# bdaiinstitute/vlfm

Hardware: NVIDIA H100
Metric: value-map steps/sec (ITM+cone-fuse) (higher is better)
Workload: dtype f16

## Files before the change

vlfm_b200/csrc/gemm_wgmma.cu:

```cuda
#include <cuda.h>
#include <cuda_fp16.h>
#include <math.h>
#include <stdlib.h>

#include "common.cuh"

namespace vlfm {

constexpr int BM = 128;
constexpr int BK = 64;
constexpr int GEMM_THREADS = 384;
constexpr int GEMM_CONSUMERS = 256;

__device__ __forceinline__ uint32_t smem_u32(const void* p) { return (uint32_t)__cvta_generic_to_shared(p); }

__device__ __forceinline__ void mbar_init(uint32_t bar, uint32_t count) {
  asm volatile("mbarrier.init.shared::cta.b64 [%0], %1;" ::"r"(bar), "r"(count));
}
__device__ __forceinline__ void mbar_expect_tx(uint32_t bar, uint32_t bytes) {
  asm volatile("mbarrier.arrive.expect_tx.shared::cta.b64 _, [%0], %1;" ::"r"(bar), "r"(bytes) : "memory");
}
__device__ __forceinline__ void mbar_arrive(uint32_t bar) {
  asm volatile("mbarrier.arrive.shared::cta.b64 _, [%0];" ::"r"(bar) : "memory");
}
// ... 59 lines not shown
    asm volatile(
        "{\n\t.reg .pred p;\n\tsetp.ne.b32 p, %66, 0;\n\t"
        "wgmma.mma_async.sync.aligned.m64n128k16.f32.f16.f16 "
        "{%0,%1,%2,%3,%4,%5,%6,%7,%8,%9,%10,%11,%12,%13,%14,%15,"
        "%16,%17,%18,%19,%20,%21,%22,%23,%24,%25,%26,%27,%28,%29,%30,%31,"
        "%32,%33,%34,%35,%36,%37,%38,%39,%40,%41,%42,%43,%44,%45,%46,%47,"
        "%48,%49,%50,%51,%52,%53,%54,%55,%56,%57,%58,%59,%60,%61,%62,%63}, %64, %65, p, 1, 1, 0, 0;\n\t}"
        : VLFM_D16(d, 0), VLFM_D16(d, 16), VLFM_D16(d, 32), VLFM_D16(d, 48) : "l"(a), "l"(b), "r"(acc));
  }
};
#undef VLFM_D16
#undef VLFM_D4

struct GemmArgs {
  const float* bias;
  void* out;
  int M, N, K, ldo, epi;
  int kb_per_split;
  long long split_stride;
  const __half* a_tail; int lda, tail_rows, tail_row0;
  void* out_lo;
  int a_box_rows;
  SplitK sk;
};
constexpr int GEMM_TAIL_MAX = 2;
static_assert(SK_SLAB_ROWS == BM + GEMM_TAIL_MAX && SK_TILE == BM, "stream-K slab = one 128 x 128 tile + its tail rows");
constexpr int GEMM_TAIL_KMAX = 6144;

__device__ __forceinline__ float gelu_erf(float x) { return 0.5f * x * (1.f + erff(x * 0.70710678118654752f)); }
__device__ __forceinline__ float silu(float x) { return x / (1.f + expf(-x)); }

__device__ __forceinline__ void epilogue_store2(const GemmArgs& g, int row, int n, float v0, float v1, bool pair, bool split) {
  const size_t idx = (size_t)row * g.ldo + n;
  if (g.epi == VLFM_EPI_BIAS_F16 || g.epi == VLFM_EPI_BIAS_GELU_F16 || g.epi == VLFM_EPI_BIAS_RELU_F16 || g.epi == VLFM_EPI_BIAS_GELU_F16X2) {
    if (g.epi == VLFM_EPI_BIAS_GELU_F16 || g.epi == VLFM_EPI_BIAS_GELU_F16X2) { v0 = gelu_erf(v0); v1 = gelu_erf(v1); }
    else if (g.epi == VLFM_EPI_BIAS_RELU_F16) { v0 = fmaxf(v0, 0.f); v1 = fmaxf(v1, 0.f); }
    __half* o = reinterpret_cast<__half*>(g.out) + idx;
    const __half2 h = __floats2half2_rn(v0, v1);
    if (pair) *reinterpret_cast<__half2*>(o) = h; else o[0] = __low2half(h);
    if (g.epi == VLFM_EPI_BIAS_GELU_F16X2) {
      const float2 f = __half22float2(h);
      const __half2 l = __floats2half2_rn((v0 - f.x) * X2_SCALE, (v1 - f.y) * X2_SCALE);
      __half* ol = reinterpret_cast<__half*>(g.out_lo) + idx;
      if (pair) *reinterpret_cast<__half2*>(ol) = l; else ol[0] = __low2half(l);
    }
  } else {
    const bool partial = (g.epi == VLFM_EPI_PARTIAL_F32);
    float* o = reinterpret_cast<float*>(g.out) + (partial ? (size_t)blockIdx.z * (size_t)g.split_stride : 0) + idx;
    if (split && !partial) {
      atomicAdd(o, v0);
// ... 418 lines not shown
        float2 sum = ld_peer_f2(off, 0);
        for (int p = 1; p < s_cl; ++p) { const float2 v = ld_peer_f2(off, p); sum.x += v.x; sum.y += v.y; }
        epilogue_store2(g, row, n, sum.x + sbias[c], sum.y + sbias[c + 1], n + 1 < g.N, false);
      }
    }
    cluster_sync_all();
  }
}

template <int BN, int STAGES>
__global__ void __launch_bounds__(GEMM_THREADS, 1)
gemm_f16x2_wgmma_kernel(const __grid_constant__ CUtensorMap tmA, const __grid_constant__ CUtensorMap tmAl,
                        const __grid_constant__ CUtensorMap tmB, const __grid_constant__ CUtensorMap tmBl, GemmArgs g) {
  constexpr uint32_t A_BYTES = BM * BK * 2, B_BYTES = BN * BK * 2;

  extern __shared__ uint8_t smem_raw[];
  uint8_t* sA = smem_align_1024(smem_raw);
  uint8_t* sAl = sA + STAGES * A_BYTES;
  uint8_t* sB = sAl + STAGES * A_BYTES;
  uint8_t* sBl = sB + STAGES * B_BYTES;
  uint64_t* bars = reinterpret_cast<uint64_t*>(sBl + STAGES * B_BYTES);
  const uint32_t full0 = smem_u32(bars), empty0 = smem_u32(bars + STAGES);
  float* sbias = reinterpret_cast<float*>(bars + 2 * STAGES);

  pdl_trigger();
  const int warp = threadIdx.x >> 5, lane = threadIdx.x & 31;
  const int n_blk = blockIdx.x, m_blk = blockIdx.y;
  const int kb_begin = blockIdx.z * g.kb_per_split;
  const int num_k = min((g.K + BK - 1) / BK - kb_begin, g.kb_per_split);
  const bool split = gridDim.z > 1;

  if (warp == 0 && lane == 0) {
    asm volatile("prefetch.tensormap [%0];" ::"l"(&tmA) : "memory");
    asm volatile("prefetch.tensormap [%0];" ::"l"(&tmAl) : "memory");
    asm volatile("prefetch.tensormap [%0];" ::"l"(&tmB) : "memory");
    asm volatile("prefetch.tensormap [%0];" ::"l"(&tmBl) : "memory");
    for (int i = 0; i < STAGES; ++i) { mbar_init(full0 + 8 * i, 1); mbar_init(empty0 + 8 * i, GEMM_CONSUMERS / 32); }
    asm volatile("fence.mbarrier_init.release.cluster;" ::: "memory");
    asm volatile("fence.proxy.async.shared::cta;" ::: "memory");
  }
  __syncthreads();

  if (warp == 0) {
    if (lane == 0) {
      const int pre = num_k < STAGES ? num_k : STAGES;
      const uint32_t a_tx = (uint32_t)g.a_box_rows * BK * 2;
      for (int kb = 0; kb < pre; ++kb) {
        mbar_expect_tx(full0 + 8 * kb, 2 * (a_tx + B_BYTES));
        tma_load_2d(smem_u32(sB + kb * B_BYTES), &tmB, (kb_begin + kb) * BK, n_blk * BN, full0 + 8 * kb);
        tma_load_2d(smem_u32(sBl + kb * B_BYTES), &tmBl, (kb_begin + kb) * BK, n_blk * BN, full0 + 8 * kb);
      }
      pdl_wait();
      for (int kb = 0; kb < pre; ++kb) {
        tma_load_2d(smem_u32(sA + kb * A_BYTES), &tmA, (kb_begin + kb) * BK, m_blk * BM, full0 + 8 * kb);
        tma_load_2d(smem_u32(sAl + kb * A_BYTES), &tmAl, (kb_begin + kb) * BK, m_blk * BM, full0 + 8 * kb);
      }
      int s = pre == STAGES ? 0 : pre; uint32_t ph = pre == STAGES ? 1 : 0;
      for (int kb = pre; kb < num_k; ++kb) {
        mbar_wait(empty0 + 8 * s, ph ^ 1);
        mbar_expect_tx(full0 + 8 * s, 2 * (a_tx + B_BYTES));
        tma_load_2d(smem_u32(sA + s * A_BYTES), &tmA, (kb_begin + kb) * BK, m_blk * BM, full0 + 8 * s);
        tma_load_2d(smem_u32(sAl + s * A_BYTES), &tmAl, (kb_begin + kb) * BK, m_blk * BM, full0 + 8 * s);
        tma_load_2d(smem_u32(sB + s * B_BYTES), &tmB, (kb_begin + kb) * BK, n_blk * BN, full0 + 8 * s);
        tma_load_2d(smem_u32(sBl + s * B_BYTES), &tmBl, (kb_begin + kb) * BK, n_blk * BN, full0 + 8 * s);
        if (++s == STAGES) { s = 0; ph ^= 1; }
      }
    }
  } else if (warp >= 4) {
    const int wg = (warp >> 2) - 1, wq = warp & 3;
    const int et = threadIdx.x - (GEMM_THREADS - GEMM_CONSUMERS);
    const int wg_row0 = m_blk * BM + wg * 64;
    const bool active = wg_row0 < g.M;
    if (et < BN) { const int n = n_blk * BN + et; sbias[et] = (g.bias && n < g.N) ? __ldg(g.bias + n) : 0.f; }
    asm volatile("bar.sync 1, 256;" ::: "memory");
    pdl_wait();
    if (!active) {
      int s = 0; uint32_t ph = 0;
      for (int kb = 0; kb < num_k; ++kb) {
        mbar_wait(full0 + 8 * s, ph);
        __syncwarp();
        if (lane == 0) mbar_arrive(empty0 + 8 * s);
        if (++s == STAGES) { s = 0; ph ^= 1; }
      }
      return;
    }
    float acc[BN / 2], corr[BN / 2];
#pragma unroll
    for (int i = 0; i < BN / 2; ++i) { acc[i] = 0.f; corr[i] = 0.f; }
    int s = 0; uint32_t ph = 0;
    for (int kb = 0; kb < num_k; ++kb) {
      mbar_wait(full0 + 8 * s, ph);
// ... 5 lines not shown
      for (int k = 0; k < BK / 16; ++k) {
        const uint64_t da = wgmma_desc_k128(a0 + k * 32), dal = wgmma_desc_k128(al0 + k * 32);
        const uint64_t db = wgmma_desc_k128(b0 + k * 32), dbl = wgmma_desc_k128(bl0 + k * 32);
        const uint32_t first = (kb > 0 || k > 0) ? 1u : 0u;
        Wgmma<BN>::mma(acc, da, db, first);
        Wgmma<BN>::mma(corr, dal, db, first);
        Wgmma<BN>::mma(corr, da, dbl, 1u);
      }
      wg_commit();
      wg_wait<1>();
      if (kb > 0) {
        __syncwarp();
        if (lane == 0) mbar_arrive(empty0 + 8 * (s == 0 ? STAGES - 1 : s - 1));
      }
      if (++s == STAGES) { s = 0; ph ^= 1; }
    }
    wg_wait<0>();
#pragma unroll
    for (int i = 0; i < BN / 2; ++i) acc[i] = fmaf(corr[i], 1.f / X2_SCALE, acc[i]);
    epilogue_frag<BN>(acc, wg_row0 + wq * 16, n_blk, g, split, blockIdx.z == 0, sbias);
  }
}

typedef CUresult (*EncodeTiledFn)(CUtensorMap*, CUtensorMapDataType, cuuint32_t, void*, const cuuint64_t*,
                                  const cuuint64_t*, const cuuint32_t*, const cuuint32_t*, CUtensorMapInterleave,
                                  CUtensorMapSwizzle, CUtensorMapL2promotion, CUtensorMapFloatOOBfill);

static EncodeTiledFn get_encode() {
  static EncodeTiledFn fn = nullptr;
  static bool tried = false;
  if (!tried) {
    tried = true;
    void* p = nullptr;
    cudaDriverEntryPointQueryResult q;
    if (cudaGetDriverEntryPoint("cuTensorMapEncodeTiled", &p, cudaEnableDefault, &q) == cudaSuccess &&
        q == cudaDriverEntryPointSuccess)
      fn = reinterpret_cast<EncodeTiledFn>(p);
  }
  return fn;
}

static int make_map(CUtensorMap* m, const void* base, int rows, int cols, int ld, int boxRows) {
  EncodeTiledFn enc = get_encode();
  if (!enc) { set_error("cuTensorMapEncodeTiled entry point unavailable"); return VLFM_E_DRIVER; }
  cuuint64_t dims[2] = {(cuuint64_t)cols, (cuuint64_t)rows};
  cuuint64_t strides[1] = {(cuuint64_t)ld * 2};
// ... 19 lines not shown
  static_assert(smem <= 227 * 1024, "GEMM stage ring exceeds the 227 KB a block may use");
  static bool configured = false;
  if (!configured) {
    rc = check_cuda(cudaFuncSetAttribute(gemm_f16_wgmma_kernel<BN, STAGES, SILU>, cudaFuncAttributeMaxDynamicSharedMemorySize, (int)smem), "cudaFuncSetAttribute(gemm)");
    if (rc) return rc;
    configured = true;
  }
  const int num_k = (g.K + BK - 1) / BK;
  dim3 grid((g.N + BN - 1) / BN, g.tail_rows > 0 ? g.M / BM : (g.M + BM - 1) / BM, (num_k + g.kb_per_split - 1) / g.kb_per_split);
  if (g.sk.ctas > 0) grid = dim3(g.sk.ctas);
  rc = check_cuda(launch_pdl(gemm_f16_wgmma_kernel<BN, STAGES, SILU>, grid, dim3(GEMM_THREADS), smem, st, ta, tb, g), "gemm_f16_wgmma_kernel");
  if (rc) return rc;
  count_launch();
  return VLFM_OK;
}


template <int BN, int STAGES>
static int launch_gemm_x2(const CUtensorMap& ta, const CUtensorMap& tal, const void* W, const void* Wl, int ldw, const GemmArgs& g, cudaStream_t st) {
  CUtensorMap tb, tbl;
  int rc = make_map(&tb, W, g.N, g.K, ldw, BN);
  if (!rc) rc = make_map(&tbl, Wl, g.N, g.K, ldw, BN);
  if (rc) return rc;
  constexpr size_t smem = (size_t)STAGES * 2 * (BM * BK * 2 + BN * BK * 2) + 2 * STAGES * 8 + 1024 + BN * 4;
  static_assert(smem <= 227 * 1024, "x2 GEMM stage ring exceeds the 227 KB a block may use");
  static bool configured = false;
  if (!configured) {
    rc = check_cuda(cudaFuncSetAttribute(gemm_f16x2_wgmma_kernel<BN, STAGES>, cudaFuncAttributeMaxDynamicSharedMemorySize, (int)smem), "cudaFuncSetAttribute(gemm x2)");
    if (rc) return rc;
    configured = true;
  }
  const int num_k = (g.K + BK - 1) / BK;
  dim3 grid((g.N + BN - 1) / BN, (g.M + BM - 1) / BM, (num_k + g.kb_per_split - 1) / g.kb_per_split);
  rc = check_cuda(launch_pdl(gemm_f16x2_wgmma_kernel<BN, STAGES>, grid, dim3(GEMM_THREADS), smem, st, ta, tal, tb, tbl, g), "gemm_f16x2_wgmma_kernel");
  if (rc) return rc;
  count_launch();
  return VLFM_OK;
}

template <int BN, int STAGES>
struct Csplit {
  static constexpr size_t smem = (size_t)STAGES * (CS_BM * BK * 2 + BN * BK * 2) + 2 * STAGES * 8 + 1024 + BN * 4 +
                                 (size_t)GEMM_TAIL_MAX * GEMM_TAIL_KMAX * 2;
  static_assert(smem <= 227 * 1024, "cluster-split GEMM stage ring exceeds the 227 KB a block may use");
  static int configure() {
    static int rc = -1;
    if (rc < 0) rc = check_cuda(cudaFuncSetAttribute(gemm_f16_csplit_wgmma_kernel<BN, STAGES>, cudaFuncAttributeMaxDynamicSharedMemorySize, (int)smem),
                                "cudaFuncSetAttribute(gemm csplit)");
    return rc;
  }
  static int max_clusters(int s) {
    static int fit[9] = {-1, -1, -1, -1, -1, -1, -1, -1, -1};
    if (fit[s] < 0) {
      fit[s] = 0;
      if (configure()) return 0;
      cudaLaunchConfig_t cfg{};
      cfg.gridDim = dim3(s); cfg.blockDim = dim3(CS_THREADS); cfg.dynamicSmemBytes = smem;
      cudaLaunchAttribute attr[1];
      attr[0].id = cudaLaunchAttributeClusterDimension;
      attr[0].val.clusterDim.x = s; attr[0].val.clusterDim.y = 1; attr[0].val.clusterDim.z = 1;
      cfg.attrs = attr; cfg.numAttrs = 1;
      int n = 0;
      if (cudaOccupancyMaxActiveClusters(&n, gemm_f16_csplit_wgmma_kernel<BN, STAGES>, &cfg) == cudaSuccess) fit[s] = n;
      else cudaGetLastError();
    }
    return fit[s];
  }
  static int launch(const CUtensorMap& ta, const void* W, int ldw, const GemmArgs& g, int s, cudaStream_t st) {
    CUtensorMap tb;
    int rc = make_map(&tb, W, g.N, g.K, ldw, BN);
    if (!rc) rc = configure();
    if (rc) return rc;
    cudaLaunchConfig_t cfg{};
    cfg.gridDim = dim3(((g.N + BN - 1) / BN) * s); cfg.blockDim = dim3(CS_THREADS); cfg.dynamicSmemBytes = smem; cfg.stream = st;
    cudaLaunchAttribute attr[2];
    attr[0].id = cudaLaunchAttributeClusterDimension;
    attr[0].val.clusterDim.x = s; attr[0].val.clusterDim.y = 1; attr[0].val.clusterDim.z = 1;
    attr[1].id = cudaLaunchAttributeProgrammaticStreamSerialization;
    attr[1].val.programmaticStreamSerializationAllowed = 1;
    cfg.attrs = attr; cfg.numAttrs = pdl_enabled() ? 2 : 1;
    rc = check_cuda(cudaLaunchKernelEx(&cfg, gemm_f16_csplit_wgmma_kernel<BN, STAGES>, ta, tb, g), "gemm_f16_csplit_wgmma_kernel");
    if (rc) return rc;
    count_launch();
    return VLFM_OK;
  }
};

}

using namespace vlfm;

static int gemm_dispatch(const void* d_A, const void* d_W, int M, int N, int K, int lda, int ldw, GemmArgs g, void* stream, float* d_partials,
                         size_t partial_bytes, SplitK* layout, bool csplit);

static int sm_count() {
  static int sms = 0;
  if (!sms) { int dev = 0; cudaGetDevice(&dev); if (cudaDeviceGetAttribute(&sms, cudaDevAttrMultiProcessorCount, dev) != cudaSuccess || sms < 1) sms = 132; }
  return sms;
}

extern "C" int vlfm_gemm_f16(const void* d_A, const void* d_W, const float* d_bias, void* d_out, int M, int N,
                             int K, int lda, int ldw, int ldo, int epilogue, void* stream) {
  if (!d_A || !d_W || !d_out || M < 1 || N < 1 || K < 1) { set_error("vlfm_gemm_f16: bad argument"); return VLFM_E_INVALID; }
  if ((K & 7) || (lda & 7) || (ldw & 7) || (ldo & 7) || ((uintptr_t)d_A & 15) || ((uintptr_t)d_W & 15) || ((uintptr_t)d_out & 15)) {
    set_error("vlfm_gemm_f16: K, lda, ldw, ldo must be multiples of 8 and pointers 16-byte aligned"); return VLFM_E_INVALID; }
  const bool csplit = (epilogue & VLFM_EPI_CLUSTER_SPLIT) != 0 && (epilogue & ~VLFM_EPI_CLUSTER_SPLIT) != VLFM_EPI_BIAS_SILU_F16;
  epilogue &= ~VLFM_EPI_CLUSTER_SPLIT;
// ... 154 lines not shown
                   int rows, int D, int ldx, int ldo16, int ldo32, float eps, void* stream);
namespace vlfm {
int layernorm_reduce_impl(float* d_x, const float* d_partials, const SplitK& sk, const float* d_gamma, const float* d_beta, void* d_out16,
                          void* d_out16_lo, float* d_out32, int rows, int D, int ldx, int ldo16, int ldo32, float eps, void* stream);
}

extern "C" int vlfm_gemm_f16_resid_ln(const void* d_A, const void* d_W, const float* d_bias, float* d_x, int M, int N, int K,
                                      int lda, int ldw, int ldx, const float* d_gamma, const float* d_beta, void* d_out16,
                                      int ld16, float* d_out32, int ld32, float eps, float* d_partials, size_t partial_bytes, void* stream) {
  if (!d_A || !d_W || !d_x || !d_gamma || !d_beta || (!d_out16 && !d_out32) || M < 1 || N < 1 || K < 1) {
    set_error("vlfm_gemm_f16_resid_ln: bad argument"); return VLFM_E_INVALID; }
  if ((K & 7) || (lda & 7) || (ldw & 7) || (ldx & 7) || (N & 3) || (ld16 & 3) || (ld32 & 3) || ((uintptr_t)d_A & 15) || ((uintptr_t)d_W & 15) ||
      ((uintptr_t)d_x & 15) || ((uintptr_t)d_partials & 15)) { set_error("vlfm_gemm_f16_resid_ln: alignment (K, strides %% 8; N %% 4; 16-byte pointers)"); return VLFM_E_INVALID; }
  int rc = layernorm_check("vlfm_gemm_f16_resid_ln", d_x, d_gamma, d_beta, d_out16, nullptr, d_out32, N, ldx, ld16, ld32);
  if (rc) return rc;
  GemmArgs g{d_bias, d_x, M, N, K, ldx, VLFM_EPI_BIAS_RESID_F32, (K + BK - 1) / BK, 0, nullptr, 0, 0, 0, nullptr, BM};
  SplitK layout;
  rc = gemm_dispatch(d_A, d_W, M, N, K, lda, ldw, g, stream, d_partials, partial_bytes, &layout, d_partials != nullptr);
  if (rc) return rc;
  if (layout.splits != 1) return layernorm_reduce_impl(d_x, d_partials, layout, d_gamma, d_beta, d_out16, nullptr, d_out32, M, N, ldx, ld16, ld32, eps, stream);
  return vlfm_layernorm(d_x, d_gamma, d_beta, d_out16, d_out32, M, N, ldx, ld16, ld32, eps, stream);
}

static int gemm_x2_dispatch(const void* d_A_hi, const void* d_A_lo, const void* d_W_hi, const void* d_W_lo, int M, int N, int K, int lda, int ldw,
                            GemmArgs g, void* stream, float* d_partials, size_t partial_bytes, int* splits_out) {
  if (splits_out) *splits_out = 1;
  const int rem = M % BM;
  if (M > BM && rem >= 1 && rem <= 32 && (g.epi == VLFM_EPI_BIAS_F32 || g.epi == VLFM_EPI_BIAS_GELU_F16X2)) {
    const int m0 = M - rem;
    GemmArgs g0 = g; g0.M = m0;
    int rc0 = gemm_x2_dispatch(d_A_hi, d_A_lo, d_W_hi, d_W_lo, m0, N, K, lda, ldw, g0, stream, nullptr, 0, nullptr);
    if (rc0) return rc0;
    GemmArgs g1 = g; g1.M = rem;
    const size_t esz = g.epi == VLFM_EPI_BIAS_F32 ? 4 : 2;
    g1.out = (uint8_t*)g.out + (size_t)m0 * g.ldo * esz;
    if (g.out_lo) g1.out_lo = (uint8_t*)g.out_lo + (size_t)m0 * g.ldo * 2;
    return gemm_x2_dispatch((const __half*)d_A_hi + (size_t)m0 * lda, (const __half*)d_A_lo + (size_t)m0 * lda, d_W_hi, d_W_lo, rem, N, K, lda, ldw, g1,
                            stream, nullptr, 0, nullptr);
  }
  CUtensorMap ta, tal;
  g.a_box_rows = M <= 32 ? 32 : (M <= 64 ? 64 : BM);
  int rc = make_map(&ta, d_A_hi, M, K, lda, g.a_box_rows);
  if (!rc) rc = make_map(&tal, d_A_lo, M, K, lda, g.a_box_rows);
  if (rc) return rc;
  const int mt = (M + BM - 1) / BM, num_k = (K + BK - 1) / BK;
  int bn = 32;
  if (mt >= 2 && N >= 4096) bn = 128;
  else if ((long)mt * ((N + 63) / 64) >= 96) bn = 64;
  const int tiles = mt * ((N + bn - 1) / bn);
  int sp = 1;
  if (g.epi == VLFM_EPI_BIAS_RESID_F32 && d_partials) {
    sp = sm_count() / tiles; if (sp > num_k / 3) sp = num_k / 3; if (sp > 8) sp = 8; if (sp < 1) sp = 1;
  }
  g.kb_per_split = (num_k + sp - 1) / sp;
  const int launched = (num_k + g.kb_per_split - 1) / g.kb_per_split;
  if (launched > 1) {
    if ((size_t)launched * (size_t)M * (size_t)N * 4 > partial_bytes) { g.kb_per_split = num_k; }
    else { g.epi = VLFM_EPI_PARTIAL_F32; g.out = d_partials; g.ldo = N; g.split_stride = (long long)M * N; if (splits_out) *splits_out = launched; }
  }
  cudaStream_t st = (cudaStream_t)stream;
  if (bn == 128) return launch_gemm_x2<128, 3>(ta, tal, d_W_hi, d_W_lo, ldw, g, st);
  if (bn == 64) return launch_gemm_x2<64, 4>(ta, tal, d_W_hi, d_W_lo, ldw, g, st);
  return launch_gemm_x2<32, 5>(ta, tal, d_W_hi, d_W_lo, ldw, g, st);
}

static int x2_args_ok(const char* who, const void* a, const void* al, const void* w, const void* wl, const void* out, int M, int N, int K, int lda, int ldw, int ldo) {
  if (!a || !al || !w || !wl || !out || M < 1 || N < 1 || K < 1) { set_error("%s: bad argument", who); return VLFM_E_INVALID; }
  if ((K & 7) || (lda & 7) || (ldw & 7) || (ldo & 7) || ((uintptr_t)a & 15) || ((uintptr_t)al & 15) || ((uintptr_t)w & 15) || ((uintptr_t)wl & 15) || ((uintptr_t)out & 15)) {
// ... 39 lines not shown
```

vlfm_b200/csrc/vit_ops.cu:

```cuda
#include <cuda_fp16.h>
#include <math.h>

#include "common.cuh"

namespace vlfm {

__device__ __forceinline__ uint8_t clip8(int v) {
  v >>= 22;
  return (uint8_t)(v < 0 ? 0 : (v > 255 ? 255 : v));
}

__global__ void resize_h_kernel(const uint8_t* __restrict__ in, uint8_t* __restrict__ mid, int H, int W, int OW,
                                const int* __restrict__ bounds, const int* __restrict__ kk, int ksize) {
  const int b = blockIdx.z, y = blockIdx.y;
  const int i = blockIdx.x * blockDim.x + threadIdx.x;
  if (i >= OW * 3) return;
  const int xo = i / 3, c = i - 3 * xo;
  const int x0 = bounds[2 * xo], n = bounds[2 * xo + 1];
  const uint8_t* row = in + ((size_t)b * H + y) * W * 3;
  int ss = 1 << 21;
  for (int t = 0; t < n; ++t) ss += (int)row[(x0 + t) * 3 + c] * kk[xo * ksize + t];
  mid[(((size_t)b * H + y) * OW + xo) * 3 + c] = clip8(ss);
}

// ... 433 lines not shown
    const float4 v = reinterpret_cast<const float4*>(src)[i];
    __half h[4], l[4];
    split_x2(v.x, h[0], l[0]); split_x2(v.y, h[1], l[1]); split_x2(v.z, h[2], l[2]); split_x2(v.w, h[3], l[3]);
    if (hi) reinterpret_cast<uint2*>(hi)[i] = *reinterpret_cast<uint2*>(h);
    reinterpret_cast<uint2*>(lo)[i] = *reinterpret_cast<uint2*>(l);
  }
}

constexpr int ATT32_NKMAX = 272;
constexpr int ATT32_KT = (ATT32_NKMAX + 31) / 32;
template <int HD>
__global__ void __launch_bounds__(256)
attention_f32_kernel(const float* __restrict__ q, const float* __restrict__ k, const float* __restrict__ v, __half* __restrict__ o_hi,
                     __half* __restrict__ o_lo, int ldq, int ldk, int ldv, int ldo, int Nq, int Nk, float scale) {
  extern __shared__ float sm32[];
  pdl_trigger();
  const int h = blockIdx.x, b = blockIdx.y, warp = threadIdx.x >> 5, lane = threadIdx.x & 31;
  constexpr int KP = HD + 1, HD4 = HD / 4, NC = HD / 32;
  float* sK = sm32;
  float* sV = sK + (((size_t)Nk * KP + 3) & ~(size_t)3);
  float* sQ = sV + (size_t)Nk * HD;
  float* sP = sQ + 8 * HD;
  pdl_wait();
  const int total = Nk * HD4;
#pragma unroll 4
  for (int i = threadIdx.x; i < total; i += 256) {
    const int j = i / HD4, c = (i - j * HD4) << 2;
    const float4 kv = __ldg(reinterpret_cast<const float4*>(k + (size_t)(b * Nk + j) * ldk + h * HD + c));
    const float4 vv = __ldg(reinterpret_cast<const float4*>(v + (size_t)(b * Nk + j) * ldv + h * HD + c));
    float* kd = sK + (size_t)j * KP + c;
    kd[0] = kv.x; kd[1] = kv.y; kd[2] = kv.z; kd[3] = kv.w;
    *reinterpret_cast<float4*>(sV + (size_t)j * HD + c) = vv;
  }
  __syncthreads();
  float* myq = sQ + warp * HD;
  float* myp = sP + (size_t)warp * Nk;
  const int kt = (Nk + 31) >> 5;
  for (int r = blockIdx.z * 8 + warp; r < Nq; r += gridDim.z * 8) {
    const float* qr = q + (size_t)(b * Nq + r) * ldq + h * HD;
#pragma unroll
    for (int c = 0; c < NC; ++c) myq[lane + 32 * c] = qr[lane + 32 * c];
    __syncwarp();
    float sc[ATT32_KT];
    const float* kr[ATT32_KT];
#pragma unroll
    for (int t = 0; t < ATT32_KT; ++t) { sc[t] = 0.f; kr[t] = sK + (size_t)min(lane + 32 * t, Nk - 1) * KP; }
#pragma unroll 4
    for (int d = 0; d < HD; ++d) {
      const float qd = myq[d];
#pragma unroll
      for (int t = 0; t < ATT32_KT; ++t) if (t < kt) sc[t] = fmaf(qd, kr[t][d], sc[t]);
    }
    float mx = -INFINITY;
#pragma unroll
    for (int t = 0; t < ATT32_KT; ++t) {
      sc[t] = (lane + 32 * t < Nk) ? sc[t] * scale : -INFINITY;
      mx = fmaxf(mx, sc[t]);
    }
#pragma unroll
    for (int o = 16; o; o >>= 1) mx = fmaxf(mx, __shfl_xor_sync(0xffffffffu, mx, o));
    float sum = 0.f;
#pragma unroll
    for (int t = 0; t < ATT32_KT; ++t) {
      const float e = (lane + 32 * t < Nk) ? expf(sc[t] - mx) : 0.f;
// ... 237 lines not shown
```

vlfm_b200/vlm/blip2_engine.py:

```python
from __future__ import annotations

import ctypes
import math
import os
from typing import Dict, List, Sequence, Tuple

import numpy as np
import torch

from .. import _lib
from . import dense
from .blip2_config import Blip2Dims
from .preprocess import CLIP_MEAN, CLIP_STD, bicubic_tables

F16, F32 = torch.float16, torch.float32


def partials_floats(dims: Blip2Dims, max_batch: int) -> int:
    rows = max_batch * dims.tokens
    return max(8 * min(rows, 1024), 3 * rows) * max(dims.v_hidden, dims.q_hidden)


class Blip2ITCEngine:
    def __init__(self, dims: Blip2Dims, state_dict: Dict[str, torch.Tensor], device="cuda", max_batch: int = 1,
# ... 158 lines not shown
        hb, hk, hks, vb, vk, vks = self._resize_tables(Hh, Ww)
        rc = self.lib.vlfm_preprocess_im2col(img.data_ptr(), mid.data_ptr(), self.b_col.data_ptr(), B, Hh, Ww, d.image, d.image,
                                             d.patch, d.patch_k_padded, hb.data_ptr(), hk.data_ptr(), hks, vb.data_ptr(),
                                             vk.data_ptr(), vks, self._mean, self._std, _lib.stream_ptr())
        _lib.check(rc, "vlfm_preprocess_im2col")
        self._gemm(self.b_col[: B * (T - 1)], self.patch_w, self.patch_b, _lib.EPI_BIAS_F32, self.b_patch[: B * (T - 1)])
        rc = self.lib.vlfm_assemble_tokens(self.b_patch.data_ptr(), self.cls.data_ptr(), self.pos.data_ptr(), self.b_x.data_ptr(),
                                           B, T, D, _lib.stream_ptr())
        _lib.check(rc, "vlfm_assemble_tokens")
        x, xn, qkv, ao, hb_ = self.b_x[:n], self.b_xn[:n], self.b_qkv[:n], self.b_ao[:n], self.b_h[:n]
        hd = D // d.v_heads
        img16, img32 = self.b_img[:n], self.b_img32[:n]
        dense.layernorm(x, self.vit[0]["ln1_w"], self.vit[0]["ln1_b"], d.v_eps, xn)
        for i, L in enumerate(self.vit):
            self._gemm(xn, L["qkv_w"], L["qkv_b"], _lib.EPI_BIAS_F16, qkv)
            dense.attention_f16(qkv[:, 0:D], qkv[:, D : 2 * D], qkv[:, 2 * D : 3 * D], B, d.v_heads, T, T, hd, hd**-0.5, ao)
            self._gemm_resid_ln(ao, L["proj_w"], L["proj_b"], x, L["ln2_w"], L["ln2_b"], xn, None, d.v_eps)
            self._gemm(xn, L["fc1_w"], L["fc1_b"], _lib.EPI_BIAS_GELU_F16, hb_)
            if i + 1 < len(self.vit):
                nx = self.vit[i + 1]
                self._gemm_resid_ln(hb_, L["fc2_w"], L["fc2_b"], x, nx["ln1_w"], nx["ln1_b"], xn, None, d.v_eps)
            else:
                self._gemm_resid_ln(hb_, L["fc2_w"], L["fc2_b"], x, self.post_w, self.post_b, img16, img32, d.v_eps)
        img_lo = self.b_img_lo[:n]
        dense.split_x2(img32, img_lo)
        kv = self.b_kv32[:n]
        self._gemm_x2(img16, img_lo, self.kv_w, self.kv_wl, self.kv_b, _lib.EPI_BIAS_F32, kv)
        h32, hhi, hlo = self.q_h32[:nq], self.q_h16[:nq], self.q_h_lo[:nq]
        h32.copy_(self.f0_32x[:nq])
        self._qformer_layers(h32, hhi, hlo, B, Q, kv, T, text=False)
        self._gemm_x2(hhi, hlo, self.vp_w, self.vp_wl, self.vp_b, _lib.EPI_BIAS_F32, self.q_proj[:nq])
        rc = self.lib.vlfm_itc_head(self.q_proj.data_ptr(), self.text_feat.data_ptr(), self.out.data_ptr(), B, Q, d.proj,
                                    _lib.stream_ptr())
        _lib.check(rc, "vlfm_itc_head")

    def _fold_layer0(self) -> None:
        d = self.d
        Q, H = d.queries, d.q_hidden
        hd = H // d.q_heads
        L = self.qf[0]
        with torch.cuda.device(self.dev):
            h32 = torch.empty(Q, H, dtype=F32, device=self.dev)
            hhi, hlo = torch.empty(Q, H, dtype=F16, device=self.dev), torch.empty(Q, H, dtype=F16, device=self.dev)
            dense.layernorm_x2(self.query_tokens, self.q_ln_w, self.q_ln_b, d.q_eps, hhi, hlo, h32)
            qkv, ahi, alo = self.q_qkv32[:Q], self.q_ao[:Q], self.q_ao_lo[:Q]
            self._gemm_x2(hhi, hlo, L["qkv_w"], L["qkv_wl"], L["qkv_b"], _lib.EPI_BIAS_F32, qkv)
# ... 99 lines not shown
```

Baseline: 227.6.

## Add cluster-split x2 GEMM for small M and fuse tail rows into x2 kernel

Adds a cluster-split K-parallel two-term fp16 (x2) GEMM kernel for M ≤ 64, which reduces partial sums across the cluster through distributed shared memory. It also lets idle producer-group warps in the main x2 kernel compute 1–2 leftover tail rows with CUDA-core FMAs, replacing a separate launch for the remainder rows. The attention kernel now loads the first query row before the K/V staging loop so that load overlaps the staging. The cost is more shared memory per block and extra mbarrier arrivals on the tail CTAs.

```diff
diff --git a/vlfm_b200/csrc/gemm_wgmma.cu b/vlfm_b200/csrc/gemm_wgmma.cu
--- a/vlfm_b200/csrc/gemm_wgmma.cu
+++ b/vlfm_b200/csrc/gemm_wgmma.cu
@@ -105,10 +105,12 @@
   void* out_lo;
   int a_box_rows;
   SplitK sk;
+  const __half* a_tail_lo;
 };
 constexpr int GEMM_TAIL_MAX = 2;
 static_assert(SK_SLAB_ROWS == BM + GEMM_TAIL_MAX && SK_TILE == BM, "stream-K slab = one 128 x 128 tile + its tail rows");
 constexpr int GEMM_TAIL_KMAX = 6144;
+constexpr int X2_TAIL_KMAX = 1536;
 
 __device__ __forceinline__ float gelu_erf(float x) { return 0.5f * x * (1.f + erff(x * 0.70710678118654752f)); }
 __device__ __forceinline__ float silu(float x) { return x / (1.f + expf(-x)); }
@@ -573,6 +575,7 @@
   uint64_t* bars = reinterpret_cast<uint64_t*>(sBl + STAGES * B_BYTES);
   const uint32_t full0 = smem_u32(bars), empty0 = smem_u32(bars + STAGES);
   float* sbias = reinterpret_cast<float*>(bars + 2 * STAGES);
+  __half* sx = reinterpret_cast<__half*>(sbias + BN);
 
   pdl_trigger();
   const int warp = threadIdx.x >> 5, lane = threadIdx.x & 31;
@@ -580,13 +583,14 @@
   const int kb_begin = blockIdx.z * g.kb_per_split;
   const int num_k = min((g.K + BK - 1) / BK - kb_begin, g.kb_per_split);
   const bool split = gridDim.z > 1;
+  const bool tail_cta = g.tail_rows > 0 && m_blk == (int)gridDim.y - 1;
 
   if (warp == 0 && lane == 0) {
     asm volatile("prefetch.tensormap [%0];" ::"l"(&tmA) : "memory");
     asm volatile("prefetch.tensormap [%0];" ::"l"(&tmAl) : "memory");
     asm volatile("prefetch.tensormap [%0];" ::"l"(&tmB) : "memory");
     asm volatile("prefetch.tensormap [%0];" ::"l"(&tmBl) : "memory");
-    for (int i = 0; i < STAGES; ++i) { mbar_init(full0 + 8 * i, 1); mbar_init(empty0 + 8 * i, GEMM_CONSUMERS / 32); }
+    for (int i = 0; i < STAGES; ++i) { mbar_init(full0 + 8 * i, 1); mbar_init(empty0 + 8 * i, GEMM_CONSUMERS / 32 + (tail_cta ? 3 : 0)); }
     asm volatile("fence.mbarrier_init.release.cluster;" ::: "memory");
     asm volatile("fence.proxy.async.shared::cta;" ::: "memory");
   }
@@ -617,7 +621,70 @@
         if (++s == STAGES) { s = 0; ph ^= 1; }
       }
     }
-  } else if (warp >= 4) {
+  } else if (warp < 4) {
+    if (!tail_cta) return;
+    const int t = threadIdx.x - 32, kpad = num_k * BK;
+    pdl_wait();
+    for (int i = t; i < g.tail_rows * 2 * (kpad >> 3); i += 96) {
+      const int rr = i / (kpad >> 3), c8 = (i - rr * (kpad >> 3)) << 3;
+      uint4 xv = make_uint4(0u, 0u, 0u, 0u);
+      if (c8 < g.K) xv = __ldg(reinterpret_cast<const uint4*>(((rr & 1) ? g.a_tail_lo : g.a_tail) + (size_t)(rr >> 1) * g.lda + c8));
+      *reinterpret_cast<uint4*>(sx + (size_t)rr * kpad + c8) = xv;
+    }
+    asm volatile("bar.sync 2, 96;" ::: "memory");
+    float tm[2][GEMM_TAIL_MAX], tc[2][GEMM_TAIL_MAX];
+#pragma unroll
+    for (int j = 0; j < 2; ++j)
+#pragma unroll
+      for (int r = 0; r < GEMM_TAIL_MAX; ++r) { tm[j][r] = 0.f; tc[j][r] = 0.f; }
+    int s = 0; uint32_t ph = 0;
+    for (int kb = 0; kb < num_k; ++kb) {
+      mbar_wait(full0 + 8 * s, ph);
+#pragma unroll
+      for (int j = 0; j < 2; ++j) {
+        const int f = t + 96 * j;
+        if (f >= BN) continue;
+        const uint8_t* wh_row = sB + (size_t)s * B_BYTES + (size_t)f * 128;
+        const uint8_t* wl_row = sBl + (size_t)s * B_BYTES + (size_t)f * 128;
+#pragma unroll 2
+        for (int c = 0; c < 8; ++c) {
+          const uint4 wh = *reinterpret_cast<const uint4*>(wh_row + ((c ^ (f & 7)) << 4));
+          const uint4 wl = *reinterpret_cast<const uint4*>(wl_row + ((c ^ (f & 7)) << 4));
+          const __half2* whh = reinterpret_cast<const __half2*>(&wh);
+          const __half2* wlh = reinterpret_cast<const __half2*>(&wl);
+#pragma unroll
+          for (int r = 0; r < GEMM_TAIL_MAX; ++r) {
+            if (r < g.tail_rows) {
+              const uint4 xh = *reinterpret_cast<const uint4*>(sx + (size_t)(2 * r) * kpad + kb * BK + c * 8);
+              const uint4 xl = *reinterpret_cast<const uint4*>(sx + (size_t)(2 * r + 1) * kpad + kb * BK + c * 8);
+              const __half2* xhh = reinterpret_cast<const __half2*>(&xh);
+              const __half2* xlh = reinterpret_cast<const __half2*>(&xl);
+#pragma unroll
+              for (int e = 0; e < 4; ++e) {
+                const float2 ah = __half22float2(xhh[e]), al = __half22float2(xlh[e]);
+                const float2 bh = __half22float2(whh[e]), bl = __half22float2(wlh[e]);
+                tm[j][r] = fmaf(ah.x, bh.x, tm[j][r]); tm[j][r] = fmaf(ah.y, bh.y, tm[j][r]);
+                tc[j][r] = fmaf(al.x, bh.x, tc[j][r]); tc[j][r] = fmaf(ah.x, bl.x, tc[j][r]);
+                tc[j][r] = fmaf(al.y, bh.y, tc[j][r]); tc[j][r] = fmaf(ah.y, bl.y, tc[j][r]);
+              }
+            }
+          }
+        }
+      }
+      __syncwarp();
+      if (lane == 0) mbar_arrive(empty0 + 8 * s);
+      if (++s == STAGES) { s = 0; ph ^= 1; }
+    }
+#pragma unroll
+    for (int j = 0; j < 2; ++j) {
+      const int f = t + 96 * j, n = n_blk * BN + f;
+      if (f >= BN || n >= g.N) continue;
+      const float b = g.bias ? __ldg(g.bias + n) : 0.f;
+#pragma unroll
+      for (int r = 0; r < GEMM_TAIL_MAX; ++r)
+        if (r < g.tail_rows) epilogue_store2(g, g.tail_row0 + r, n, fmaf(tc[j][r], 1.f / X2_SCALE, tm[j][r]) + b, 0.f, false, false);
+    }
+  } else {
     const int wg = (warp >> 2) - 1, wq = warp & 3;
     const int et = threadIdx.x - (GEMM_THREADS - GEMM_CONSUMERS);
     const int wg_row0 = m_blk * BM + wg * 64;
@@ -669,6 +736,136 @@
   }
 }
 
+constexpr int CX_THREADS = 256;
+constexpr int CX_ROWS = 64;
+
+template <int BN, int STAGES>
+__global__ void __launch_bounds__(CX_THREADS, 1)
+gemm_f16x2_csplit_wgmma_kernel(const __grid_constant__ CUtensorMap tmA, const __grid_constant__ CUtensorMap tmAl,
+                         const __grid_constant__ CUtensorMap tmB, const __grid_constant__ CUtensorMap tmBl, GemmArgs g) {
+  constexpr uint32_t A_BYTES = CX_ROWS * BK * 2, B_BYTES = BN * BK * 2;
+  constexpr int LDP = BN + 8;
+  static_assert((size_t)CX_ROWS * LDP * 4 <= (size_t)STAGES * 2 * (A_BYTES + B_BYTES), "partial tile must fit the ring");
+
+  extern __shared__ uint8_t smem_raw[];
+  uint8_t* sA = smem_align_1024(smem_raw);
+  uint8_t* sAl = sA + STAGES * A_BYTES;
+  uint8_t* sB = sAl + STAGES * A_BYTES;
+  uint8_t* sBl = sB + STAGES * B_BYTES;
+  uint64_t* bars = reinterpret_cast<uint64_t*>(sBl + STAGES * B_BYTES);
+  const uint32_t full0 = smem_u32(bars), empty0 = smem_u32(bars + STAGES);
+  float* sbias = reinterpret_cast<float*>(bars + 2 * STAGES);
+  float* part = reinterpret_cast<float*>(sA);
+
+  pdl_trigger();
+  const int warp = threadIdx.x >> 5, lane = threadIdx.x & 31;
+  const int nk = (g.K + BK - 1) / BK;
+  const int s_cl = (int)cluster_nctarank(), rank = (int)cluster_ctarank();
+  const int n_blk = blockIdx.x / s_cl;
+  const int kb_lo = rank * nk / s_cl, kb_hi = (rank + 1) * nk / s_cl;
+
+  if (warp == 0 && lane == 0) {
+    asm volatile("prefetch.tensormap [%0];" ::"l"(&tmA) : "memory");
+    asm volatile("prefetch.tensormap [%0];" ::"l"(&tmAl) : "memory");
+    asm volatile("prefetch.tensormap [%0];" ::"l"(&tmB) : "memory");
+    asm volatile("prefetch.tensormap [%0];" ::"l"(&tmBl) : "memory");
+    for (int i = 0; i < STAGES; ++i) { mbar_init(full0 + 8 * i, 1); mbar_init(empty0 + 8 * i, 4); }
+    asm volatile("fence.mbarrier_init.release.cluster;" ::: "memory");
+    asm volatile("fence.proxy.async.shared::cta;" ::: "memory");
+  }
+  __syncthreads();
+
+  if (warp < 4) {
+    if (warp == 0 && lane == 0) {
+      const int pre = min(kb_hi - kb_lo, STAGES);
+      const uint32_t tx = 2 * ((uint32_t)g.a_box_rows * BK * 2 + B_BYTES);
+      for (int i = 0; i < pre; ++i) {
+        mbar_expect_tx(full0 + 8 * i, tx);
+        tma_load_2d(smem_u32(sB + i * B_BYTES), &tmB, (kb_lo + i) * BK, n_blk * BN, full0 + 8 * i);
+        tma_load_2d(smem_u32(sBl + i * B_BYTES), &tmBl, (kb_lo + i) * BK, n_blk * BN, full0 + 8 * i);
+      }
+      pdl_wait();
+      for (int i = 0; i < pre; ++i) {
+        tma_load_2d(smem_u32(sA + i * A_BYTES), &tmA, (kb_lo + i) * BK, 0, full0 + 8 * i);
+        tma_load_2d(smem_u32(sAl + i * A_BYTES), &tmAl, (kb_lo + i) * BK, 0, full0 + 8 * i);
+      }
+      int s = pre == STAGES ? 0 : pre; uint32_t ph = pre == STAGES ? 1 : 0;
+      for (int kb = kb_lo + pre; kb < kb_hi; ++kb) {
+        mbar_wait(empty0 + 8 * s, ph ^ 1);
+        mbar_expect_tx(full0 + 8 * s, tx);
+        tma_load_2d(smem_u32(sA + s * A_BYTES), &tmA, kb * BK, 0, full0 + 8 * s);
+        tma_load_2d(smem_u32(sAl + s * A_BYTES), &tmAl, kb * BK, 0, full0 + 8 * s);
+        tma_load_2d(smem_u32(sB + s * B_BYTES), &tmB, kb * BK, n_blk * BN, full0 + 8 * s);
+        tma_load_2d(smem_u32(sBl + s * B_BYTES), &tmBl, kb * BK, n_blk * BN, full0 + 8 * s);
+        if (++s == STAGES) { s = 0; ph ^= 1; }
+      }
+    }
+    __syncwarp();
+  } else {
+    const int wq = warp & 3, et = threadIdx.x - 128;
+    if (et < BN) { const int n = n_blk * BN + et; sbias[et] = (g.bias && n < g.N) ? __ldg(g.bias + n) : 0.f; }
+    asm volatile("bar.sync 1, 128;" ::: "memory");
+    pdl_wait();
+    float acc[BN / 2], corr[BN / 2];
+#pragma unroll
+    for (int i = 0; i < BN / 2; ++i) { acc[i] = 0.f; corr[i] = 0.f; }
+    int s = 0; uint32_t ph = 0;
+    for (int kb = kb_lo; kb < kb_hi; ++kb) {
+      mbar_wait(full0 + 8 * s, ph);
+      const uint32_t a0 = smem_u32(sA + s * A_BYTES), al0 = smem_u32(sAl + s * A_BYTES);
+      const uint32_t b0 = smem_u32(sB + s * B_BYTES), bl0 = smem_u32(sBl + s * B_BYTES);
+      wg_fence();
+#pragma unroll
+      for (int k = 0; k < BK / 16; ++k) {
+        const uint64_t da = wgmma_desc_k128(a0 + k * 32), dal = wgmma_desc_k128(al0 + k * 32);
+        const uint64_t db = wgmma_desc_k128(b0 + k * 32), dbl = wgmma_desc_k128(bl0 + k * 32);
+        const uint32_t first = (kb > kb_lo || k > 0) ? 1u : 0u;
+        Wgmma<BN>::mma(acc, da, db, first);
+        Wgmma<BN>::mma(corr, dal, db, first);
+        Wgmma<BN>::mma(corr, da, dbl, 1u);
+      }
+      wg_commit();
+      wg_wait<1>();
+      if (kb > kb_lo) {
+        __syncwarp();
+        if (lane == 0) mbar_arrive(empty0 + 8 * (s == 0 ? STAGES - 1 : s - 1));
+      }
+      if (++s == STAGES) { s = 0; ph ^= 1; }
+    }
+    wg_wait<0>();
+#pragma unroll
+    for (int i = 0; i < BN / 2; ++i) acc[i] = fmaf(corr[i], 1.f / X2_SCALE, acc[i]);
+    if (s_cl == 1) {
+      epilogue_frag<BN>(acc, wq * 16, n_blk, g, false, true, sbias);
+    } else {
+      asm volatile("bar.sync 1, 128;" ::: "memory");
+      const int r_up = wq * 16 + (lane >> 2), cq = (lane & 3) * 2;
+#pragma unroll
+      for (int j = 0; j < BN / 8; ++j) {
+        *reinterpret_cast<float2*>(part + r_up * LDP + j * 8 + cq) = make_float2(acc[4 * j], acc[4 * j + 1]);
+        *reinterpret_cast<float2*>(part + (r_up + 8) * LDP + j * 8 + cq) = make_float2(acc[4 * j + 2], acc[4 * j + 3]);
+      }
+    }
+  }
+  if (s_cl > 1) {
+    cluster_sync_all();
+    if (warp >= 4) {
+      const int et = threadIdx.x - 128;
+      const int r0 = rank * g.M / s_cl, r1 = (rank + 1) * g.M / s_cl;
+      const uint32_t base = smem_u32(part);
+      for (int i = et; i < (r1 - r0) * (BN / 2); i += 128) {
+        const int row = r0 + i / (BN / 2), c = (i % (BN / 2)) * 2, n = n_blk * BN + c;
+        if (n >= g.N) continue;
+        const uint32_t off = base + (uint32_t)(row * LDP + c) * 4;
+        float2 sum = ld_peer_f2(off, 0);
+        for (int p = 1; p < s_cl; ++p) { const float2 v = ld_peer_f2(off, p); sum.x += v.x; sum.y += v.y; }
+        epilogue_store2(g, row, n, sum.x + sbias[c], sum.y + sbias[c + 1], n + 1 < g.N, false);
+      }
+    }
+    cluster_sync_all();
+  }
+}
+
 typedef CUresult (*EncodeTiledFn)(CUtensorMap*, CUtensorMapDataType, cuuint32_t, void*, const cuuint64_t*,
                                   const cuuint64_t*, const cuuint32_t*, const cuuint32_t*, CUtensorMapInterleave,
                                   CUtensorMapSwizzle, CUtensorMapL2promotion, CUtensorMapFloatOOBfill);
@@ -734,7 +931,8 @@
   int rc = make_map(&tb, W, g.N, g.K, ldw, BN);
   if (!rc) rc = make_map(&tbl, Wl, g.N, g.K, ldw, BN);
   if (rc) return rc;
-  constexpr size_t smem = (size_t)STAGES * 2 * (BM * BK * 2 + BN * BK * 2) + 2 * STAGES * 8 + 1024 + BN * 4;
+  constexpr size_t smem = (size_t)STAGES * 2 * (BM * BK * 2 + BN * BK * 2) + 2 * STAGES * 8 + 1024 + BN * 4 +
+                          (size_t)2 * GEMM_TAIL_MAX * X2_TAIL_KMAX * 2;
   static_assert(smem <= 227 * 1024, "x2 GEMM stage ring exceeds the 227 KB a block may use");
   static bool configured = false;
   if (!configured) {
@@ -743,58 +941,88 @@
     configured = true;
   }
   const int num_k = (g.K + BK - 1) / BK;
-  dim3 grid((g.N + BN - 1) / BN, (g.M + BM - 1) / BM, (num_k + g.kb_per_split - 1) / g.kb_per_split);
+  dim3 grid((g.N + BN - 1) / BN, g.tail_rows > 0 ? g.M / BM : (g.M + BM - 1) / BM, (num_k + g.kb_per_split - 1) / g.kb_per_split);
   rc = check_cuda(launch_pdl(gemm_f16x2_wgmma_kernel<BN, STAGES>, grid, dim3(GEMM_THREADS), smem, st, ta, tal, tb, tbl, g), "gemm_f16x2_wgmma_kernel");
   if (rc) return rc;
   count_launch();
   return VLFM_OK;
 }
 
-template <int BN, int STAGES>
-struct Csplit {
-  static constexpr size_t smem = (size_t)STAGES * (CS_BM * BK * 2 + BN * BK * 2) + 2 * STAGES * 8 + 1024 + BN * 4 +
-                                 (size_t)GEMM_TAIL_MAX * GEMM_TAIL_KMAX * 2;
-  static_assert(smem <= 227 * 1024, "cluster-split GEMM stage ring exceeds the 227 KB a block may use");
-  static int configure() {
-    static int rc = -1;
-    if (rc < 0) rc = check_cuda(cudaFuncSetAttribute(gemm_f16_csplit_wgmma_kernel<BN, STAGES>, cudaFuncAttributeMaxDynamicSharedMemorySize, (int)smem),
-                                "cudaFuncSetAttribute(gemm csplit)");
-    return rc;
-  }
-  static int max_clusters(int s) {
-    static int fit[9] = {-1, -1, -1, -1, -1, -1, -1, -1, -1};
+template <typename Kernel>
+struct ClusterLaunch {
+  Kernel kernel; int threads; size_t smem; const char* name;
+  int configure(int* state) const {
+    if (*state < 0) *state = check_cuda(cudaFuncSetAttribute(kernel, cudaFuncAttributeMaxDynamicSharedMemorySize, (int)smem), name);
+    return *state;
+  }
+  int max_clusters(int s, int* fit, int* state) const {
     if (fit[s] < 0) {
       fit[s] = 0;
-      if (configure()) return 0;
+      if (configure(state)) return 0;
       cudaLaunchConfig_t cfg{};
-      cfg.gridDim = dim3(s); cfg.blockDim = dim3(CS_THREADS); cfg.dynamicSmemBytes = smem;
+      cfg.gridDim = dim3(s); cfg.blockDim = dim3(threads); cfg.dynamicSmemBytes = smem;
       cudaLaunchAttribute attr[1];
       attr[0].id = cudaLaunchAttributeClusterDimension;
       attr[0].val.clusterDim.x = s; attr[0].val.clusterDim.y = 1; attr[0].val.clusterDim.z = 1;
       cfg.attrs = attr; cfg.numAttrs = 1;
       int n = 0;
-      if (cudaOccupancyMaxActiveClusters(&n, gemm_f16_csplit_wgmma_kernel<BN, STAGES>, &cfg) == cudaSuccess) fit[s] = n;
+      if (cudaOccupancyMaxActiveClusters(&n, kernel, &cfg) == cudaSuccess) fit[s] = n;
       else cudaGetLastError();
     }
     return fit[s];
   }
-  static int launch(const CUtensorMap& ta, const void* W, int ldw, const GemmArgs& g, int s, cudaStream_t st) {
-    CUtensorMap tb;
-    int rc = make_map(&tb, W, g.N, g.K, ldw, BN);
-    if (!rc) rc = configure();
+  template <typename... Args>
+  int launch(int col_tiles, int s, cudaStream_t st, int* state, const Args&... args) const {
+    int rc = configure(state);
     if (rc) return rc;
     cudaLaunchConfig_t cfg{};
-    cfg.gridDim = dim3(((g.N + BN - 1) / BN) * s); cfg.blockDim = dim3(CS_THREADS); cfg.dynamicSmemBytes = smem; cfg.stream = st;
+    cfg.gridDim = dim3(col_tiles * s); cfg.blockDim = dim3(threads); cfg.dynamicSmemBytes = smem; cfg.stream = st;
     cudaLaunchAttribute attr[2];
     attr[0].id = cudaLaunchAttributeClusterDimension;
     attr[0].val.clusterDim.x = s; attr[0].val.clusterDim.y = 1; attr[0].val.clusterDim.z = 1;
     attr[1].id = cudaLaunchAttributeProgrammaticStreamSerialization;
     attr[1].val.programmaticStreamSerializationAllowed = 1;
     cfg.attrs = attr; cfg.numAttrs = pdl_enabled() ? 2 : 1;
-    rc = check_cuda(cudaLaunchKernelEx(&cfg, gemm_f16_csplit_wgmma_kernel<BN, STAGES>, ta, tb, g), "gemm_f16_csplit_wgmma_kernel");
+    rc = check_cuda(cudaLaunchKernelEx(&cfg, kernel, args...), name);
     if (rc) return rc;
     count_launch();
     return VLFM_OK;
+  }
+};
+
+template <int BN, int STAGES>
+struct Csplit {
+  static constexpr size_t smem = (size_t)STAGES * (CS_BM * BK * 2 + BN * BK * 2) + 2 * STAGES * 8 + 1024 + BN * 4 +
+                                 (size_t)GEMM_TAIL_MAX * GEMM_TAIL_KMAX * 2;
+  static_assert(smem <= 227 * 1024, "cluster-split GEMM stage ring exceeds the 227 KB a block may use");
+  static inline int state = -1, fit[9] = {-1, -1, -1, -1, -1, -1, -1, -1, -1};
+  static ClusterLaunch<decltype(&gemm_f16_csplit_wgmma_kernel<BN, STAGES>)> kl() {
+    return {gemm_f16_csplit_wgmma_kernel<BN, STAGES>, CS_THREADS, smem, "gemm_f16_csplit_wgmma_kernel"};
+  }
+  static int max_clusters(int s) { return kl().max_clusters(s, fit, &state); }
+  static int launch(const CUtensorMap& ta, const void* W, int ldw, const GemmArgs& g, int s, cudaStream_t st) {
+    CUtensorMap tb;
+    int rc = make_map(&tb, W, g.N, g.K, ldw, BN);
+    if (rc) return rc;
+    return kl().launch((g.N + BN - 1) / BN, s, st, &state, ta, tb, g);
+  }
+};
+
+template <int BN, int STAGES>
+struct CsplitX2 {
+  static constexpr size_t smem = (size_t)STAGES * 2 * (CX_ROWS * BK * 2 + BN * BK * 2) + 2 * STAGES * 8 + 1024 + BN * 4;
+  static_assert(smem <= 227 * 1024, "cluster-split x2 GEMM stage ring exceeds the 227 KB a block may use");
+  static inline int state = -1, fit[9] = {-1, -1, -1, -1, -1, -1, -1, -1, -1};
+  static ClusterLaunch<decltype(&gemm_f16x2_csplit_wgmma_kernel<BN, STAGES>)> kl() {
+    return {gemm_f16x2_csplit_wgmma_kernel<BN, STAGES>, CX_THREADS, smem, "gemm_f16x2_csplit_wgmma_kernel"};
+  }
+  static int max_clusters(int s) { return kl().max_clusters(s, fit, &state); }
+  static int launch(const CUtensorMap& ta, const CUtensorMap& tal, const void* W, const void* Wl, int ldw, const GemmArgs& g, int s, cudaStream_t st) {
+    CUtensorMap tb, tbl;
+    int rc = make_map(&tb, W, g.N, g.K, ldw, BN);
+    if (!rc) rc = make_map(&tbl, Wl, g.N, g.K, ldw, BN);
+    if (rc) return rc;
+    return kl().launch((g.N + BN - 1) / BN, s, st, &state, ta, tal, tb, tbl, g);
   }
 };
 
@@ -995,11 +1223,36 @@
   return vlfm_layernorm(d_x, d_gamma, d_beta, d_out16, d_out32, M, N, ldx, ld16, ld32, eps, stream);
 }
 
+constexpr int CX_STAGES = 5;
+static int csplit_x2_fit(int bn, int s) {
+  return bn == 64 ? CsplitX2<64, CX_STAGES>::max_clusters(s) : CsplitX2<32, CX_STAGES>::max_clusters(s);
+}
+static CsplitPlan csplit_x2_plan(int M, int N, int K, int box_rows) {
+  const int nk = (K + BK - 1) / BK;
+  CsplitPlan best{0, 0, 0.0};
+  bool best_fits = false;
+  const int bns[2] = {64, 32};
+  for (int bn : bns) {
+    const int nt = (N + bn - 1) / bn;
+    for (int s = 1; s <= 8 && s <= nk; ++s) {
+      if (nt > csplit_x2_fit(bn, s)) continue;
+      const int kb = (nk + s - 1) / s;
+      const bool fits = kb <= CX_STAGES;
+      double bytes = (double)kb * 2 * (box_rows + bn) * BK * 2;
+      if (s > 1) bytes += (double)(s - 1) / s * M * bn * 4 + CS_RED_FIXED_BYTES;
+      if (!best.bn || (fits && !best_fits) || (fits == best_fits && bytes < best.cta_bytes)) { best = CsplitPlan{bn, s, bytes}; best_fits = fits; }
+    }
+  }
+  return best;
+}
+
 static int gemm_x2_dispatch(const void* d_A_hi, const void* d_A_lo, const void* d_W_hi, const void* d_W_lo, int M, int N, int K, int lda, int ldw,
                             GemmArgs g, void* stream, float* d_partials, size_t partial_bytes, int* splits_out) {
   if (splits_out) *splits_out = 1;
   const int rem = M % BM;
-  if (M > BM && rem >= 1 && rem <= 32 && (g.epi == VLFM_EPI_BIAS_F32 || g.epi == VLFM_EPI_BIAS_GELU_F16X2)) {
+  const bool unsplit_epi = g.epi == VLFM_EPI_BIAS_F32 || g.epi == VLFM_EPI_BIAS_GELU_F16X2;
+  const bool tail = M > BM && rem >= 1 && rem <= GEMM_TAIL_MAX && K <= X2_TAIL_KMAX && unsplit_epi;
+  if (!tail && M > BM && rem >= 1 && rem <= 32 && unsplit_epi) {
     const int m0 = M - rem;
     GemmArgs g0 = g; g0.M = m0;
     int rc0 = gemm_x2_dispatch(d_A_hi, d_A_lo, d_W_hi, d_W_lo, m0, N, K, lda, ldw, g0, stream, nullptr, 0, nullptr);
@@ -1016,7 +1269,19 @@
   int rc = make_map(&ta, d_A_hi, M, K, lda, g.a_box_rows);
   if (!rc) rc = make_map(&tal, d_A_lo, M, K, lda, g.a_box_rows);
   if (rc) return rc;
-  const int mt = (M + BM - 1) / BM, num_k = (K + BK - 1) / BK;
+  if (M <= CX_ROWS) {
+    const CsplitPlan p = csplit_x2_plan(M, N, K, g.a_box_rows);
+    if (p.bn) {
+      cudaStream_t cst = (cudaStream_t)stream;
+      if (p.bn == 64) return CsplitX2<64, CX_STAGES>::launch(ta, tal, d_W_hi, d_W_lo, ldw, g, p.s, cst);
+      return CsplitX2<32, CX_STAGES>::launch(ta, tal, d_W_hi, d_W_lo, ldw, g, p.s, cst);
+    }
+  }
+  if (tail) {
+    g.a_tail = (const __half*)d_A_hi + (size_t)(M - rem) * lda; g.a_tail_lo = (const __half*)d_A_lo + (size_t)(M - rem) * lda;
+    g.lda = lda; g.tail_rows = rem; g.tail_row0 = M - rem;
+  }
+  const int mt = tail ? M / BM : (M + BM - 1) / BM, num_k = (K + BK - 1) / BK;
   int bn = 32;
   if (mt >= 2 && N >= 4096) bn = 128;
   else if ((long)mt * ((N + 63) / 64) >= 96) bn = 64;
diff --git a/vlfm_b200/csrc/vit_ops.cu b/vlfm_b200/csrc/vit_ops.cu
--- a/vlfm_b200/csrc/vit_ops.cu
+++ b/vlfm_b200/csrc/vit_ops.cu
@@ -479,8 +479,17 @@
   float* sQ = sV + (size_t)Nk * HD;
   float* sP = sQ + 8 * HD;
   pdl_wait();
+  float* myq = sQ + warp * HD;
+  {
+    const int r = blockIdx.z * 8 + warp;
+    if (r < Nq) {
+      const float* qr = q + (size_t)(b * Nq + r) * ldq + h * HD;
+#pragma unroll
+      for (int c = 0; c < NC; ++c) myq[lane + 32 * c] = qr[lane + 32 * c];
+    }
+  }
   const int total = Nk * HD4;
-#pragma unroll 4
+#pragma unroll 8
   for (int i = threadIdx.x; i < total; i += 256) {
     const int j = i / HD4, c = (i - j * HD4) << 2;
     const float4 kv = __ldg(reinterpret_cast<const float4*>(k + (size_t)(b * Nk + j) * ldk + h * HD + c));
@@ -490,13 +499,14 @@
     *reinterpret_cast<float4*>(sV + (size_t)j * HD + c) = vv;
   }
   __syncthreads();
-  float* myq = sQ + warp * HD;
   float* myp = sP + (size_t)warp * Nk;
   const int kt = (Nk + 31) >> 5;
   for (int r = blockIdx.z * 8 + warp; r < Nq; r += gridDim.z * 8) {
-    const float* qr = q + (size_t)(b * Nq + r) * ldq + h * HD;
-#pragma unroll
-    for (int c = 0; c < NC; ++c) myq[lane + 32 * c] = qr[lane + 32 * c];
+    if (r != blockIdx.z * 8 + warp) {
+      const float* qr = q + (size_t)(b * Nq + r) * ldq + h * HD;
+#pragma unroll
+      for (int c = 0; c < NC; ++c) myq[lane + 32 * c] = qr[lane + 32 * c];
+    }
     __syncwarp();
     float sc[ATT32_KT];
     const float* kr[ATT32_KT];
diff --git a/vlfm_b200/vlm/blip2_engine.py b/vlfm_b200/vlm/blip2_engine.py
--- a/vlfm_b200/vlm/blip2_engine.py
+++ b/vlfm_b200/vlm/blip2_engine.py
@@ -204,6 +204,13 @@
                 self._gemm_resid_ln(hb_, L["fc2_w"], L["fc2_b"], x, nx["ln1_w"], nx["ln1_b"], xn, None, d.v_eps)
             else:
                 self._gemm_resid_ln(hb_, L["fc2_w"], L["fc2_b"], x, self.post_w, self.post_b, img16, img32, d.v_eps)
+        self._qformer_impl(B)
+
+    def _qformer_impl(self, B: int) -> None:
+        d = self.d
+        T, Q = d.tokens, d.queries
+        n, nq = B * T, B * Q
+        img16, img32 = self.b_img[:n], self.b_img32[:n]
         img_lo = self.b_img_lo[:n]
         dense.split_x2(img32, img_lo)
         kv = self.b_kv32[:n]
```

New measurement: 230.8 (median of 6 runs). 1.01x the previous value.
